# dougsouza/pytorch-sync-batchnorm-example

Hardware: AMD Instinct MI355X
Metric: images/sec (whole node) resnet50 SyncBN (higher is better)
Workload: dtype bf16; 1 GPU; model=resnet50, global_batch=512, per_gpu_batch=512, image=3x224x224, memory_format=channels_last, parallelism=dp1, impl=msbn, hip_graph=False, conv_autotune=False, fused_bn_act=True

## Files before the change

### msbn/models/resnet.py

```python

from typing import List, Type, Union

import torch
import torch.nn as nn

from msbn.nn import BatchNorm2d, SyncBatchNorm
from msbn.nn.fused import SyncBatchNormAct2d


def conv3x3(cin, cout, stride=1):
    return nn.Conv2d(cin, cout, 3, stride=stride, padding=1, bias=False)


def conv1x1(cin, cout, stride=1):
    return nn.Conv2d(cin, cout, 1, stride=stride, bias=False)


def _norm(planes, fused):
    return SyncBatchNorm(planes) if fused else BatchNorm2d(planes)


def _split(x):
    return x if isinstance(x, tuple) else (x, x)

# ... 77 lines not shown


class ResNet(nn.Module):
    def __init__(
        self,
        block: Type[Union[BasicBlock, Bottleneck]],
        layers: List[int],
        num_classes: int = 1000,
        in_chans: int = 3,
        fused: bool = False,
        fork_grads: bool = True,
    ):
        super().__init__()
        self.fused = fused
        self.fork_grads = fork_grads and fused
        self.inplanes = 64
        self.conv1 = nn.Conv2d(in_chans, 64, 7, stride=2, padding=3, bias=False)
        if fused:
            self.bn1 = SyncBatchNormAct2d(64, relu=True)
        else:
            self.bn1 = BatchNorm2d(64)
        self.relu = nn.ReLU(inplace=True)
        self.maxpool = nn.MaxPool2d(3, stride=2, padding=1)
        self.layer1 = self._make_layer(block, 64, layers[0])
        self.layer2 = self._make_layer(block, 128, layers[1], stride=2)
        self.layer3 = self._make_layer(block, 256, layers[2], stride=2)
        self.layer4 = self._make_layer(block, 512, layers[3], stride=2,
                                       fork_last=False)
        self.avgpool = nn.AdaptiveAvgPool2d(1)
        self.fc = nn.Linear(512 * block.expansion, num_classes)
# ... 10 lines not shown
            downsample = nn.Sequential(
                conv1x1(self.inplanes, planes * block.expansion, stride),
                _norm(planes * block.expansion, self.fused),
            )
        layers = [block(self.inplanes, planes, stride, downsample,
                        fused=self.fused, fork=fork[0])]
        self.inplanes = planes * block.expansion
        for i in range(1, blocks):
            layers.append(block(self.inplanes, planes, fused=self.fused,
                                fork=fork[i]))
        return nn.Sequential(*layers)

    def _stem(self, x):
        x = self.conv1(x)
        if self.fused:
            return self.maxpool(self.bn1(x))
        return self.maxpool(self.relu(self.bn1(x)))

    def forward_features(self, x):
        x = self._stem(x)
        c2 = self.layer1(x)
        c3 = self.layer2(c2)
        c4 = self.layer3(c3)
        c5 = self.layer4(c4)
        return _split(c2)[0], _split(c3)[0], _split(c4)[0], _split(c5)[0]

    def forward(self, x):
        _, _, _, c5 = self.forward_features(x)
        out = self.avgpool(c5).flatten(1)
        return self.fc(out)
# ... 13 lines not shown
```

### msbn/nn/fused.py

```python

from typing import Optional

import torch
import torch.distributed as dist

from msbn import ops
from msbn.nn.batchnorm import (SyncBatchNorm, _check_negative_slope,
                               _momentum_factor, _running_stats_forward)
from msbn.nn.functions import (_combined_view, _contig, _force_sync,
                               _match_layout, compute_sync_stats)


class SyncBatchNormActFunction(torch.autograd.Function):
    @staticmethod
    def forward(
        ctx,
        input: torch.Tensor,
        residual: Optional[torch.Tensor],
        weight: Optional[torch.Tensor],
        bias: Optional[torch.Tensor],
        running_mean: Optional[torch.Tensor],
        running_var: Optional[torch.Tensor],
        eps: float,
        momentum: float,
# ... 183 lines not shown
            else:
                grad_input, grad_res = ops.batch_norm_backward_elemt_act(
                    grad_output, input, residual, mean, invstd, weight, bias,
                    sum_dy, sum_dy_xmu, count_sum, relu, need_res_g, coefs,
                    slope,
                )
        return (
            grad_input if need_input_g else None,
            grad_res,
            grad_weight if need_weight_g else None,
            grad_bias if need_bias_g else None,
            None, None, None, None, None, None, None, None, None,
        )


class InPlaceSyncBatchNormActFunction(torch.autograd.Function):

    @staticmethod
    def forward(
        ctx,
        input: torch.Tensor,
        weight: torch.Tensor,
        bias: torch.Tensor,
        running_mean: Optional[torch.Tensor],
        running_var: Optional[torch.Tensor],
        eps: float,
        momentum: float,
        process_group,
        world_size: int,
        act: bool,
# ... 172 lines not shown
```

### msbn/ops/__init__.py

```python

from typing import Optional

import torch

from msbn.ops import _reference as _ref

_C = None
_C_IMPORT_ERROR: Optional[BaseException] = None
try:
    import os as _os

    if _os.environ.get("MSBN_AB_NONT", "0") == "1":
        from msbn import _C_nont as _C
    else:
        from msbn import _C as _C
except Exception as e:
    _C_IMPORT_ERROR = e


def hip_available() -> bool:
    return _C is not None


def _require_hip():
# ... 185 lines not shown
                                  relu_mask, want_res_grad, coefs=None,
                                  negative_slope: float = 0.0):
    if input.is_cuda:
        dx, dres = _require_hip().batch_norm_backward_elemt_act(
            grad_out, input, residual, mean, invstd, weight, bias, sum_dy,
            sum_dy_xmu, count, relu_mask, want_res_grad, coefs,
            negative_slope,
        )
        return dx, (dres if want_res_grad else None)
    return _ref.batch_norm_backward_elemt_act(
        grad_out, input, residual, mean, invstd, weight, bias, sum_dy,
        sum_dy_xmu, count, relu_mask, want_res_grad, negative_slope,
    )


def batch_norm_elemt_act_(input, weight, bias, mean, invstd, act: bool,
                          coefs=None, negative_slope: float = 0.0):
    if input.is_cuda:
        _require_hip().batch_norm_elemt_act_(
            input, weight, bias, mean, invstd, act, coefs, negative_slope
        )
        return input
    return _ref.batch_norm_elemt_act_(
        input, weight, bias, mean, invstd, act, negative_slope
    )


def batch_norm_backward_reduce_inplace(grad_out, output, invstd, weight, bias,
                                       act: bool, input_g, weight_g, bias_g,
                                       coefs=None,
# ... 51 lines not shown

def launch_plan(kind: str, input: torch.Tensor, others=(), coefs=None) -> dict:
    path, numbers = _require_hip().launch_plan(kind, input, list(others), coefs)
    plan = dict(numbers)
    plan["path"] = path
    if "multi_trip" in plan:
        plan["multi_trip"] = bool(plan["multi_trip"])
    return plan


__all__ = [
    "hip_available",
    "launch_plan",
    "bn_frozen_coefs",
    "batch_norm_frozen_backward_elemt",
    "batch_norm_elemt_act_",
    "batch_norm_backward_reduce_inplace",
    "batch_norm_backward_elemt_inplace",
    "batch_norm_elemt_act",
    "bn_make_coefs",
    "batch_norm_backward_reduce_act",
    "batch_norm_backward_elemt_act",
    "batch_norm_stats",
    "batch_norm_stats_packed",
    "batch_norm_gather_stats_with_counts",
    "batch_norm_gather_stats_packed",
    "batch_norm_elemt",
    "batch_norm_backward_reduce",
    "batch_norm_backward_elemt",
]
# ... 1 lines not shown
```

### msbn/ops/_reference.py

```python

from typing import Optional, Tuple

import torch


def _flatten_to_ncs(input: torch.Tensor) -> torch.Tensor:
    if input.dim() == 2:
        return input.unsqueeze(-1)
    return input.reshape(input.shape[0], input.shape[1], -1)


def batch_norm_stats(input: torch.Tensor, eps: float) -> Tuple[torch.Tensor, torch.Tensor]:
    x = _flatten_to_ncs(input)
    C = x.shape[1]
    n = x.shape[0] * x.shape[2]
    if n == 0:
        z = torch.zeros(C, dtype=torch.float32, device=input.device)
        return z, z.clone()
    xd = x.transpose(0, 1).reshape(C, -1).to(torch.float64)
    mean = xd.mean(dim=1)
    var = xd.var(dim=1, unbiased=False)
    invstd = torch.rsqrt(var + eps)
    return mean.to(torch.float32), invstd.to(torch.float32)

# ... 128 lines not shown

def batch_norm_backward_elemt_act(
    grad_out, input, residual, mean, invstd, weight, bias, sum_dy,
    sum_dy_xmu, count, relu_mask, want_res_grad, negative_slope: float = 0.0,
):
    g = _masked_grad(grad_out, input, residual, mean, invstd, weight, bias,
                     relu_mask, negative_slope)
    dx = batch_norm_backward_elemt(
        g, input, mean, invstd, weight, sum_dy, sum_dy_xmu, count
    )
    dres = g.to(grad_out.dtype) if want_res_grad else None
    return dx, dres



def _check_invertible(act: bool, negative_slope: float, name: str):
    if act and not negative_slope > 0.0:
        raise RuntimeError(
            f"{name}: the in-place path needs an invertible activation "
            "(identity, or LeakyReLU with negative_slope > 0); got "
            f"negative_slope={negative_slope}"
        )


def _slope32(negative_slope: float):
    s = torch.tensor(negative_slope, dtype=torch.float32)
    return s, 1.0 / s


def _invert_act(grad_out, output, act: bool, negative_slope: float):
# ... 144 lines not shown
```

### msbn/ops/csrc/bn_kernels.hip

```cpp
#include "bn_ops.hpp"
#include "common.hpp"

#include <ATen/ATen.h>
#include <c10/hip/HIPStream.h>

#include <algorithm>
#include <map>
#include <string>
#include <vector>

namespace msbn {

namespace {

template <typename T, int V>
__global__ void bn_stats_partial_nchw(const T* __restrict__ x,
                                      double* __restrict__ ws, int64_t N,
                                      int64_t C, int64_t S, int64_t chunkN,
                                      int64_t chunkS) {
  const int64_t c = blockIdx.x;
  const int64_t n0 = blockIdx.y * chunkN;
  const int64_t n1 = i64min(n0 + chunkN, N);
  const int64_t s0 = blockIdx.z * chunkS;
  const int64_t s1 = i64min(s0 + chunkS, S);
// ... 1375 lines not shown
      float g = to_f(nt_load1(&dy[e])), z;
      inv_act<ACT>(to_f(nt_load1(&y[e])), g, z, slope, inv_slope);
      nt_store1(&dx[e], from_f<T>(ca[c] * g + cb[c] * z + cd[c]));
    } else {
      Pack<T, V> pg = nt_load<T, V>(&dy[e]);
      Pack<T, V> py = nt_load<T, V>(&y[e]);
      Pack<float, V> pa = *reinterpret_cast<const Pack<float, V>*>(&ca[c]);
      Pack<float, V> pb = *reinterpret_cast<const Pack<float, V>*>(&cb[c]);
      Pack<float, V> pd = *reinterpret_cast<const Pack<float, V>*>(&cd[c]);
      Pack<T, V> po;
#pragma unroll
      for (int k = 0; k < V; ++k) {
        float g = to_f(pg.v[k]), z;
        inv_act<ACT>(to_f(py.v[k]), g, z, slope, inv_slope);
        po.v[k] = from_f<T>(pa.v[k] * g + pb.v[k] * z + pd.v[k]);
      }
      nt_store<T, V>(&dx[e], po);
    }
  }
}


struct Layout {
  bool nhwc;
  int64_t N, C, S;
  int64_t rows;
};

Layout get_layout(const at::Tensor& t) {
  Layout L{};
// ... 892 lines not shown
  });
  return {dx, dres};
}

at::Tensor batch_norm_backward_elemt(
    const at::Tensor& grad_out, const at::Tensor& input, const at::Tensor& mean,
    const at::Tensor& invstd, const c10::optional<at::Tensor>& weight,
    const at::Tensor& sum_dy, const at::Tensor& sum_dy_xmu,
    const at::Tensor& count) {
  return std::get<0>(batch_norm_backward_elemt_act(
      grad_out, input, c10::nullopt, mean, invstd, weight, c10::nullopt,
      sum_dy, sum_dy_xmu, count, false, false, c10::nullopt, 0.0));
}

namespace {
int inplace_act_mode(bool act, float slope, const char* name) {
  TORCH_CHECK(!act || slope > 0.f, name,
              ": the in-place path needs an invertible activation (identity, "
              "or LeakyReLU with negative_slope > 0); got negative_slope=",
              slope);
  return act ? kActLeaky : kActNone;
}

void check_same_dense(const at::Tensor& a, const at::Tensor& ref,
                      const char* what) {
  TORCH_CHECK(a.sizes() == ref.sizes() && a.strides() == ref.strides() &&
                  a.scalar_type() == ref.scalar_type() &&
                  a.device() == ref.device(),
              what, " must match the output's shape/strides/dtype/device");
}
// ... 580 lines not shown
  std::string path;

  if (kind == "fused_local") {
    if (!bn_fused_local_eligible(input, c10::nullopt, c10::nullopt,
                                 c10::nullopt, c10::nullopt))
      return {"ineligible", d};
    const int64_t C = input.size(1);
    const int64_t plane = input.numel() / C;
    const int64_t S = plane / input.size(0);
    d["V"] = pick_v(esize, ptrs, S);
    d["trips"] = cdiv(plane / d["V"], MSBN_BLOCK);
    d["blocks"] = C;
    return {"small_plane", d};
  }

  const Layout L = get_layout(input);
  if (kind == "stats" || kind == "bwd_reduce" ||
      kind == "bwd_reduce_inplace") {
    const ReducePlan p = plan_reduce(L, esize, ptrs);
    path = p.path == RedPath::Nhwc       ? "nhwc"
           : p.path == RedPath::NchwFlat ? "nchw_flat"
                                         : "nchw_vec";
    d["V"] = p.v;
    d["nchunks"] = p.nchunks;
    d["trips"] = p.trips;
    d["flush_every"] = p.flush_every;
    d["finalize_trips"] = cdiv(p.nchunks, MSBN_WAVE);
    if (p.path == RedPath::NchwVec) {
      d["chunkN"] = p.nchw.chunkN;
      d["chunkS"] = p.nchw.chunkS;
      d["nchunkS"] = p.nchw.grid.z;
    } else if (p.path == RedPath::NchwFlat) {
      d["chunk_len"] = p.flat.chunk_len;
    } else {
      d["chunk_rows"] = p.nhwc.chunk_rows;
      d["lpr"] = p.nhwc.lpr;
      d["ctiles"] = p.nhwc.grid.x;
    }
    return {path, d};
  }
  TORCH_CHECK(kind == "elemt" || kind == "bwd_elemt" ||
                  kind == "frozen_bwd_elemt" || kind == "elemt_inplace" ||
                  kind == "bwd_elemt_inplace",
              "launch_plan: unknown kind '", kind, "'");
  const ElemtPlan p = plan_elemt(L, input.numel(), esize, ptrs, coef);
  path = L.nhwc ? "nhwc" : (p.v == 1 ? "nchw_flat" : "nchw_vec");
  const int64_t threads = (int64_t)p.grid * MSBN_BLOCK;
  d["V"] = p.v;
  d["grid"] = p.grid;
  d["packs"] = p.packs;
  d["trips"] = cdiv(p.packs, threads);
  d["multi_trip"] = p.packs > threads ? 1 : 0;
  return {path, d};
}

}
```

### msbn/ops/csrc/bn_ops.hpp

```cpp
#pragma once

#include <ATen/ATen.h>

#include <map>
#include <string>
#include <tuple>
#include <vector>

namespace msbn {

std::tuple<at::Tensor, at::Tensor> batch_norm_stats(const at::Tensor& input,
                                                    double eps);

void batch_norm_stats_packed(const at::Tensor& input, double eps,
                             at::Tensor& out);

std::tuple<at::Tensor, at::Tensor> batch_norm_gather_stats_with_counts(
    const at::Tensor& mean_all, const at::Tensor& invstd_all,
    const c10::optional<at::Tensor>& running_mean,
    const c10::optional<at::Tensor>& running_var, double momentum, double eps,
    const at::Tensor& counts);

std::tuple<at::Tensor, at::Tensor, at::Tensor> batch_norm_gather_stats_packed(
    const at::Tensor& packed_all, const c10::optional<at::Tensor>& running_mean,
// ... 88 lines not shown
                           const at::Tensor& mean, const at::Tensor& invstd,
                           const c10::optional<at::Tensor>& weight,
                           const c10::optional<at::Tensor>& coefs,
                           bool relu_mask, bool want_res_grad, bool weight_g,
                           bool bias_g, double negative_slope);

std::tuple<at::Tensor, at::Tensor> batch_norm_backward_elemt_act(
    const at::Tensor& grad_out, const at::Tensor& input,
    const c10::optional<at::Tensor>& residual, const at::Tensor& mean,
    const at::Tensor& invstd, const c10::optional<at::Tensor>& weight,
    const c10::optional<at::Tensor>& bias, const at::Tensor& sum_dy,
    const at::Tensor& sum_dy_xmu, const at::Tensor& count, bool relu_mask,
    bool want_res_grad, const c10::optional<at::Tensor>& coefs_in,
    double negative_slope);

at::Tensor batch_norm_elemt_act_(at::Tensor& input,
                                 const c10::optional<at::Tensor>& weight,
                                 const c10::optional<at::Tensor>& bias,
                                 const at::Tensor& mean,
                                 const at::Tensor& invstd, bool act,
                                 const c10::optional<at::Tensor>& coefs_in,
                                 double negative_slope);

std::tuple<at::Tensor, at::Tensor, at::Tensor, at::Tensor>
batch_norm_backward_reduce_inplace(
    const at::Tensor& grad_out, const at::Tensor& output,
    const at::Tensor& invstd, const c10::optional<at::Tensor>& weight,
    const c10::optional<at::Tensor>& bias, bool act, bool input_g,
    bool weight_g, bool bias_g, const c10::optional<at::Tensor>& coefs_in,
    double negative_slope);
// ... 16 lines not shown
```

### msbn/ops/csrc/common.hpp

```cpp
#pragma once

#include <hip/hip_runtime.h>
#include <hip/hip_bf16.h>
#include <hip/hip_fp16.h>

#define MSBN_WAVE 64
#define MSBN_BLOCK 256

namespace msbn {

template <typename T, int V>
struct alignas(sizeof(T) * V) Pack {
  T v[V];
};

__device__ __forceinline__ float to_f(float x) { return x; }
__device__ __forceinline__ float to_f(__hip_bfloat16 x) {
  return __bfloat162float(x);
}
__device__ __forceinline__ float to_f(__half x) { return __half2float(x); }

template <typename T>
__device__ __forceinline__ T from_f(float x);
template <>
// ... 38 lines not shown
template <>
struct NTVec<16> {
  using type = int __attribute__((vector_size(16)));
};
template <>
struct NTVec<8> {
  using type = int __attribute__((vector_size(8)));
};
template <>
struct NTVec<4> {
  using type = int;
};
template <>
struct NTVec<2> {
  using type = short;
};

template <typename T, int V>
__device__ __forceinline__ Pack<T, V> nt_load(const T* p) {
#ifdef MSBN_DISABLE_NT
  return *reinterpret_cast<const Pack<T, V>*>(p);
#else
  using VT = typename NTVec<(int)sizeof(T) * V>::type;
  union {
    VT v;
    Pack<T, V> pk;
  } u;
  u.v = __builtin_nontemporal_load(reinterpret_cast<const VT*>(p));
  return u.pk;
#endif
// ... 97 lines not shown
```

### msbn/ops/csrc/module.cpp

```cpp
#include <torch/extension.h>

#include <torch/csrc/distributed/c10d/ProcessGroup.hpp>

#include "bn_ops.hpp"
#include "reducer.hpp"

PYBIND11_MODULE(TORCH_EXTENSION_NAME, m) {
  m.doc() = "msbn MI355X-native kernels + reducer";

  m.def("batch_norm_stats", &msbn::batch_norm_stats, py::arg("input"),
        py::arg("eps"));
  m.def("batch_norm_stats_packed", &msbn::batch_norm_stats_packed,
        py::arg("input"), py::arg("eps"), py::arg("out"));
  m.def("batch_norm_gather_stats_with_counts",
        &msbn::batch_norm_gather_stats_with_counts, py::arg("mean_all"),
        py::arg("invstd_all"), py::arg("running_mean"), py::arg("running_var"),
        py::arg("momentum"), py::arg("eps"), py::arg("counts"));
  m.def("batch_norm_gather_stats_packed",
        &msbn::batch_norm_gather_stats_packed, py::arg("packed_all"),
        py::arg("running_mean"), py::arg("running_var"), py::arg("momentum"),
        py::arg("eps"));
  m.def("batch_norm_gather_stats_packed_coefs",
        &msbn::batch_norm_gather_stats_packed_coefs, py::arg("packed_all"),
        py::arg("running_mean"), py::arg("running_var"), py::arg("momentum"),
// ... 22 lines not shown
        py::arg("coefs") = py::none(), py::arg("negative_slope") = 0.0);
  m.def("batch_norm_backward_reduce_act",
        &msbn::batch_norm_backward_reduce_act, py::arg("grad_out"),
        py::arg("input"), py::arg("residual"), py::arg("mean"),
        py::arg("invstd"), py::arg("weight"), py::arg("bias"),
        py::arg("relu_mask"), py::arg("input_g"), py::arg("weight_g"),
        py::arg("bias_g"), py::arg("coefs") = py::none(),
        py::arg("gm_out") = py::none(), py::arg("negative_slope") = 0.0,
        py::arg("grad_out2") = py::none());
  m.def("batch_norm_backward_elemt_act", &msbn::batch_norm_backward_elemt_act,
        py::arg("grad_out"), py::arg("input"), py::arg("residual"),
        py::arg("mean"), py::arg("invstd"), py::arg("weight"), py::arg("bias"),
        py::arg("sum_dy"), py::arg("sum_dy_xmu"), py::arg("count"),
        py::arg("relu_mask"), py::arg("want_res_grad"),
        py::arg("coefs") = py::none(), py::arg("negative_slope") = 0.0);

  m.def("batch_norm_elemt_act_", &msbn::batch_norm_elemt_act_,
        py::arg("input"), py::arg("weight"), py::arg("bias"), py::arg("mean"),
        py::arg("invstd"), py::arg("act"), py::arg("coefs") = py::none(),
        py::arg("negative_slope") = 0.0);
  m.def("batch_norm_backward_reduce_inplace",
        &msbn::batch_norm_backward_reduce_inplace, py::arg("grad_out"),
        py::arg("output"), py::arg("invstd"), py::arg("weight"),
        py::arg("bias"), py::arg("act"), py::arg("input_g"),
        py::arg("weight_g"), py::arg("bias_g"), py::arg("coefs") = py::none(),
        py::arg("negative_slope") = 0.0);
  m.def("batch_norm_backward_elemt_inplace",
        &msbn::batch_norm_backward_elemt_inplace, py::arg("grad_out"),
        py::arg("output"), py::arg("mean"), py::arg("invstd"),
        py::arg("weight"), py::arg("bias"), py::arg("sum_dy"),
// ... 71 lines not shown
```

Measured before the change: 9520 images/sec.

## Fuse stem BN+ReLU with 3x3 maxpool using argmax codes in forward and backward

```diff
diff --git a/msbn/models/resnet.py b/msbn/models/resnet.py
--- a/msbn/models/resnet.py
+++ b/msbn/models/resnet.py
@@ -5,7 +5,7 @@
 import torch.nn as nn
 
 from msbn.nn import BatchNorm2d, SyncBatchNorm
-from msbn.nn.fused import SyncBatchNormAct2d
+from msbn.nn.fused import SyncBatchNormAct2d, bn_act_maxpool
 
 
 def conv3x3(cin, cout, stride=1):
@@ -115,6 +115,7 @@
         super().__init__()
         self.fused = fused
         self.fork_grads = fork_grads and fused
+        self.stem_pool = fused
         self.inplanes = 64
         self.conv1 = nn.Conv2d(in_chans, 64, 7, stride=2, padding=3, bias=False)
         if fused:
@@ -155,6 +156,10 @@
     def _stem(self, x):
         x = self.conv1(x)
         if self.fused:
+            if (getattr(self, "stem_pool", True)
+                    and isinstance(self.bn1, SyncBatchNormAct2d)):
+                return bn_act_maxpool(self.bn1, self.maxpool, x,
+                                      fork=getattr(self, "fork_grads", False))
             return self.maxpool(self.bn1(x))
         return self.maxpool(self.relu(self.bn1(x)))
 
diff --git a/msbn/nn/fused.py b/msbn/nn/fused.py
--- a/msbn/nn/fused.py
+++ b/msbn/nn/fused.py
@@ -221,6 +221,155 @@
         )
 
 
+class SyncBatchNormActPoolFunction(torch.autograd.Function):
+
+    @staticmethod
+    def forward(
+        ctx,
+        input: torch.Tensor,
+        weight: Optional[torch.Tensor],
+        bias: Optional[torch.Tensor],
+        running_mean: Optional[torch.Tensor],
+        running_var: Optional[torch.Tensor],
+        eps: float,
+        momentum: float,
+        process_group,
+        world_size: int,
+        relu: bool,
+        negative_slope: float = 0.0,
+        fork: bool = False,
+    ):
+        if weight is not None:
+            weight = weight.contiguous()
+        if bias is not None:
+            bias = bias.contiguous()
+        use_sync = world_size > 1 or (
+            process_group is not None and _force_sync()
+        )
+        mean, invstd, count_sum, coefs = compute_sync_stats(
+            input, eps, momentum, running_mean, running_var,
+            process_group, world_size, weight, bias, want_coefs=True,
+        )
+        pooled, codes = ops.batch_norm_elemt_act_pool(
+            input, weight, bias, mean, invstd, relu, coefs, negative_slope
+        )
+        ctx.has_coefs = coefs is not None
+        saved = (input, codes, weight, bias, mean, invstd, count_sum)
+        ctx.save_for_backward(*(saved + ((coefs,) if ctx.has_coefs else ())))
+        ctx.relu = relu
+        ctx.negative_slope = negative_slope
+        ctx.process_group = process_group
+        ctx.use_sync = use_sync
+        if not fork:
+            return pooled
+        ctx.set_materialize_grads(False)
+        return pooled, pooled.detach()
+
+    @staticmethod
+    def backward(ctx, grad_output, grad_skip=None):
+        if grad_output is None:
+            grad_output, grad_skip = grad_skip, None
+        if grad_output is None:
+            return (None,) * 12
+        saved = ctx.saved_tensors
+        input, codes, weight, bias, mean, invstd, count_sum = saved[:7]
+        coefs = saved[7] if ctx.has_coefs else None
+        grad_output = _match_layout(grad_output, codes)
+        if grad_skip is not None:
+            grad_skip = _match_layout(grad_skip, codes)
+        relu, slope = ctx.relu, ctx.negative_slope
+        process_group = ctx.process_group
+        need_input_g = ctx.needs_input_grad[0]
+        need_weight_g = weight is not None and ctx.needs_input_grad[1]
+        need_bias_g = bias is not None and ctx.needs_input_grad[2]
+        C = int(input.shape[1])
+
+        sum_dy, sum_dy_xmu, grad_weight, grad_bias = (
+            ops.batch_norm_backward_reduce_act_pool(
+                grad_output, grad_skip, codes, input, mean, invstd, weight,
+                bias, relu, need_input_g, need_weight_g, need_bias_g, coefs,
+                slope,
+            )
+        )
+        grad_input = None
+        if need_input_g:
+            if ctx.use_sync:
+                combined, copied = _combined_view(sum_dy, sum_dy_xmu, C)
+                from msbn.utils import debug as _dbg
+                if _dbg.enabled():
+                    _dbg.verify_collective("syncbn.bwd.all_reduce",
+                                           combined, process_group)
+                dist.all_reduce(combined, dist.ReduceOp.SUM,
+                                group=process_group)
+                from msbn.utils.logging import comm_log
+                comm_log.record("all_reduce", combined.numel() * 4,
+                                f"syncbn bwd C={C}")
+                if copied:
+                    sum_dy, sum_dy_xmu = combined[:C], combined[C:]
+            grad_input = ops.batch_norm_backward_elemt_act_pool(
+                grad_output, grad_skip, codes, input, mean, invstd, weight,
+                bias, sum_dy, sum_dy_xmu, count_sum, relu, coefs, slope,
+            )
+        return (
+            grad_input,
+            grad_weight if need_weight_g else None,
+            grad_bias if need_bias_g else None,
+            None, None, None, None, None, None, None, None, None,
+        )
+
+
+def stem_pool_eligible(bn, pool, input: torch.Tensor) -> bool:
+    def _pair(v):
+        return tuple(v) if isinstance(v, (tuple, list)) else (v, v)
+
+    def _hooked(m):
+        return bool(m._forward_hooks or m._forward_pre_hooks
+                    or m._backward_hooks or m._backward_pre_hooks)
+
+    return (
+        type(bn) is SyncBatchNormAct2d
+        and not getattr(bn, "inplace", False)
+        and not _hooked(bn) and not _hooked(pool)
+        and (bn.training
+             or (bn.running_mean is None and bn.running_var is None))
+        and type(pool) is torch.nn.MaxPool2d
+        and _pair(pool.kernel_size) == (3, 3)
+        and _pair(pool.stride) == (2, 2)
+        and _pair(pool.padding) == (1, 1)
+        and _pair(pool.dilation) == (1, 1)
+        and not pool.ceil_mode and not pool.return_indices
+        and input.is_cuda and input.dim() == 4 and input.numel() > 0
+        and input.is_contiguous(memory_format=torch.channels_last)
+        and input.dtype in (torch.float32, torch.bfloat16, torch.float16)
+    )
+
+
+def bn_act_maxpool(bn, pool, input: torch.Tensor, fork: bool = False):
+    if not stem_pool_eligible(bn, pool, input):
+        y = pool(bn(input))
+        return (y, y) if fork else y
+    bn._check_input_dim(input)
+    bn._check_non_zero_input_channels(input)
+    if bn.training and bn.track_running_stats:
+        if bn.num_batches_tracked is not None:
+            bn.num_batches_tracked.add_(1)
+    factor = _momentum_factor(bn) if bn.training else (
+        bn.momentum if bn.momentum is not None else 0.0
+    )
+    process_group = None
+    world_size = 1
+    if dist.is_available() and dist.is_initialized():
+        process_group = bn.process_group or dist.group.WORLD
+        world_size = dist.get_world_size(process_group)
+    running_mean = bn.running_mean if bn.track_running_stats else None
+    running_var = bn.running_var if bn.track_running_stats else None
+    return SyncBatchNormActPoolFunction.apply(
+        input, bn.weight, bn.bias, running_mean, running_var, bn.eps, factor,
+        process_group, world_size, bn.relu,
+        getattr(bn, "negative_slope", 0.0), fork,
+    )
+
+
 class InPlaceSyncBatchNormActFunction(torch.autograd.Function):
 
     @staticmethod
diff --git a/msbn/ops/__init__.py b/msbn/ops/__init__.py
--- a/msbn/ops/__init__.py
+++ b/msbn/ops/__init__.py
@@ -223,6 +223,48 @@
     )
 
 
+def batch_norm_elemt_act_pool(input, weight, bias, mean, invstd, relu: bool,
+                              coefs=None, negative_slope: float = 0.0):
+    if input.is_cuda:
+        return _require_hip().batch_norm_elemt_act_pool(
+            input, weight, bias, mean, invstd, relu, coefs, negative_slope
+        )
+    return _ref.batch_norm_elemt_act_pool(
+        input, weight, bias, mean, invstd, relu, negative_slope
+    )
+
+
+def batch_norm_backward_reduce_act_pool(grad_out, grad_out2, codes, input,
+                                        mean, invstd, weight, bias, relu_mask,
+                                        input_g, weight_g, bias_g, coefs=None,
+                                        negative_slope: float = 0.0):
+    if input.is_cuda:
+        return _require_hip().batch_norm_backward_reduce_act_pool(
+            grad_out, grad_out2, codes, input, mean, invstd, weight, bias,
+            relu_mask, input_g, weight_g, bias_g, coefs, negative_slope,
+        )
+    return _ref.batch_norm_backward_reduce_act_pool(
+        grad_out, grad_out2, codes, input, mean, invstd, weight, bias,
+        relu_mask, input_g, weight_g, bias_g, negative_slope,
+    )
+
+
+def batch_norm_backward_elemt_act_pool(grad_out, grad_out2, codes, input,
+                                       mean, invstd, weight, bias, sum_dy,
+                                       sum_dy_xmu, count, relu_mask,
+                                       coefs=None,
+                                       negative_slope: float = 0.0):
+    if input.is_cuda:
+        return _require_hip().batch_norm_backward_elemt_act_pool(
+            grad_out, grad_out2, codes, input, mean, invstd, weight, bias,
+            sum_dy, sum_dy_xmu, count, relu_mask, coefs, negative_slope,
+        )
+    return _ref.batch_norm_backward_elemt_act_pool(
+        grad_out, grad_out2, codes, input, mean, invstd, weight, bias,
+        sum_dy, sum_dy_xmu, count, relu_mask, negative_slope,
+    )
+
+
 def batch_norm_elemt_act_(input, weight, bias, mean, invstd, act: bool,
                           coefs=None, negative_slope: float = 0.0):
     if input.is_cuda:
@@ -304,6 +346,9 @@
     "launch_plan",
     "bn_frozen_coefs",
     "batch_norm_frozen_backward_elemt",
+    "batch_norm_elemt_act_pool",
+    "batch_norm_backward_reduce_act_pool",
+    "batch_norm_backward_elemt_act_pool",
     "batch_norm_elemt_act_",
     "batch_norm_backward_reduce_inplace",
     "batch_norm_backward_elemt_inplace",
diff --git a/msbn/ops/_reference.py b/msbn/ops/_reference.py
--- a/msbn/ops/_reference.py
+++ b/msbn/ops/_reference.py
@@ -166,6 +166,106 @@
 
 
 
+def pool_out_size(size: int) -> int:
+    return (size - 1) // 2 + 1
+
+
+def _pooled_like(t: torch.Tensor, ref: torch.Tensor) -> torch.Tensor:
+    if ref.is_contiguous(memory_format=torch.channels_last):
+        return t.contiguous(memory_format=torch.channels_last)
+    return t.contiguous()
+
+
+def batch_norm_elemt_act_pool(input, weight, bias, mean, invstd, relu: bool,
+                              negative_slope: float = 0.0):
+    y = batch_norm_elemt_act(input, None, weight, bias, mean, invstd, relu,
+                             negative_slope)
+    N, C, H, W = y.shape
+    OH, OW = pool_out_size(H), pool_out_size(W)
+    yp = torch.nn.functional.pad(y.to(torch.float32), (1, 1, 1, 1),
+                                 value=float("-inf"))
+    best = torch.full((N, C, OH, OW), float("-inf"), dtype=torch.float32,
+                      device=y.device)
+    first_h = torch.zeros(OH, dtype=torch.uint8, device=y.device)
+    first_w = torch.zeros(OW, dtype=torch.uint8, device=y.device)
+    first_h[0] = 3
+    first_w[0] = 1
+    codes = (first_h.reshape(1, 1, OH, 1) + first_w.reshape(1, 1, 1, OW)
+             ).expand(N, C, OH, OW).clone()
+    for kh in range(3):
+        for kw in range(3):
+            val = yp[:, :, kh:kh + 2 * OH - 1:2, kw:kw + 2 * OW - 1:2]
+            upd = (val > best) | torch.isnan(val)
+            best = torch.where(upd, val, best)
+            codes = torch.where(upd, torch.full_like(codes, kh * 3 + kw),
+                                codes)
+    return (_pooled_like(best.to(input.dtype), input),
+            _pooled_like(codes, input))
+
+
+def pool_codes_to_indices(codes: torch.Tensor, H: int, W: int) -> torch.Tensor:
+    OH, OW = codes.shape[2], codes.shape[3]
+    c = codes.to(torch.int64)
+    oh = torch.arange(OH, device=codes.device).reshape(1, 1, OH, 1)
+    ow = torch.arange(OW, device=codes.device).reshape(1, 1, 1, OW)
+    return (2 * oh - 1 + c // 3) * W + (2 * ow - 1 + c % 3)
+
+
+def pool_gather_grad(grad_out, grad_out2, codes, input):
+    g = grad_out
+    if grad_out2 is not None:
+        g = grad_out + grad_out2
+    g = g.to(torch.float32)
+    N, C, H, W = input.shape
+    OH, OW = codes.shape[2], codes.shape[3]
+    full = torch.zeros((N, C, H, W), dtype=torch.float32,
+                       device=input.device)
+    for kh in (2, 1, 0):
+        lo_h = 1 if kh == 0 else 0
+        hi_h = min(OH - 1, (H - kh) // 2)
+        for kw in (2, 1, 0):
+            lo_w = 1 if kw == 0 else 0
+            hi_w = min(OW - 1, (W - kw) // 2)
+            if hi_h < lo_h or hi_w < lo_w:
+                continue
+            sel = (slice(None), slice(None), slice(lo_h, hi_h + 1),
+                   slice(lo_w, hi_w + 1))
+            part = torch.where(codes[sel] == kh * 3 + kw, g[sel],
+                               torch.zeros_like(g[sel]))
+            h0, w0 = 2 * lo_h - 1 + kh, 2 * lo_w - 1 + kw
+            dst = (slice(None), slice(None),
+                   slice(h0, h0 + 2 * (hi_h - lo_h) + 1, 2),
+                   slice(w0, w0 + 2 * (hi_w - lo_w) + 1, 2))
+            full[dst] = full[dst] + part
+    full = full.to(input.dtype)
+    if input.is_contiguous(memory_format=torch.channels_last):
+        full = full.contiguous(memory_format=torch.channels_last)
+    return full
+
+
+def batch_norm_backward_reduce_act_pool(
+    grad_out, grad_out2, codes, input, mean, invstd, weight, bias, relu_mask,
+    input_g, weight_g, bias_g, negative_slope: float = 0.0,
+):
+    g = pool_gather_grad(grad_out, grad_out2, codes, input)
+    return batch_norm_backward_reduce_act(
+        g, input, None, mean, invstd, weight, bias, relu_mask, input_g,
+        weight_g, bias_g, None, negative_slope,
+    )
+
+
+def batch_norm_backward_elemt_act_pool(
+    grad_out, grad_out2, codes, input, mean, invstd, weight, bias, sum_dy,
+    sum_dy_xmu, count, relu_mask, negative_slope: float = 0.0,
+):
+    g = pool_gather_grad(grad_out, grad_out2, codes, input)
+    return batch_norm_backward_elemt_act(
+        g, input, None, mean, invstd, weight, bias, sum_dy, sum_dy_xmu,
+        count, relu_mask, False, negative_slope,
+    )[0]
+
+
+
 def _check_invertible(act: bool, negative_slope: float, name: str):
     if act and not negative_slope > 0.0:
         raise RuntimeError(
diff --git a/msbn/ops/csrc/bn_kernels.hip b/msbn/ops/csrc/bn_kernels.hip
--- a/msbn/ops/csrc/bn_kernels.hip
+++ b/msbn/ops/csrc/bn_kernels.hip
@@ -1413,6 +1413,300 @@
         float g = to_f(pg.v[k]), z;
         inv_act<ACT>(to_f(py.v[k]), g, z, slope, inv_slope);
         po.v[k] = from_f<T>(pa.v[k] * g + pb.v[k] * z + pd.v[k]);
+      }
+      nt_store<T, V>(&dx[e], po);
+    }
+  }
+}
+
+#ifndef MSBN_POOL_FWD_NT
+#define MSBN_POOL_FWD_NT 0
+#endif
+#ifndef MSBN_POOL_GATHER_NT
+#define MSBN_POOL_GATHER_NT 0
+#endif
+
+template <typename T, int V, bool NT>
+__device__ __forceinline__ Pack<T, V> pool_load(const T* p) {
+  if (NT) return nt_load<T, V>(p);
+  return *reinterpret_cast<const Pack<T, V>*>(p);
+}
+
+template <typename T, int V, int ACT>
+__global__ void bn_elemt_pool_nhwc(const T* __restrict__ x,
+                                   T* __restrict__ y,
+                                   uint8_t* __restrict__ codes,
+                                   const float* __restrict__ scale,
+                                   const float* __restrict__ shift,
+                                   int64_t total, int64_t C, int H, int W,
+                                   int OH, int OW, float slope) {
+  const int64_t stride = (int64_t)gridDim.x * blockDim.x;
+  for (int64_t i = (int64_t)blockIdx.x * blockDim.x + threadIdx.x;
+       i * V < total; i += stride) {
+    const int64_t e = i * V;
+    const uint32_t pix = (uint32_t)(e / C);
+    const int64_t c = e - (int64_t)pix * C;
+    const uint32_t t = pix / (uint32_t)OW;
+    const int ow = (int)(pix - t * (uint32_t)OW);
+    const int n = (int)(t / (uint32_t)OH);
+    const int oh = (int)(t - (uint32_t)n * (uint32_t)OH);
+    const int h0 = 2 * oh - 1, w0 = 2 * ow - 1;
+    Pack<float, V> ps, pb;
+    if (V == 1) {
+      ps.v[0] = scale[c];
+      pb.v[0] = shift[c];
+    } else {
+      ps = *reinterpret_cast<const Pack<float, V>*>(&scale[c]);
+      pb = *reinterpret_cast<const Pack<float, V>*>(&shift[c]);
+    }
+    float best[V];
+    uint8_t code[V];
+    const uint8_t first = (uint8_t)((h0 < 0 ? 3 : 0) + (w0 < 0 ? 1 : 0));
+#pragma unroll
+    for (int k = 0; k < V; ++k) {
+      best[k] = -INFINITY;
+      code[k] = first;
+    }
+#pragma unroll
+    for (int kh = 0; kh < 3; ++kh) {
+      const int h = h0 + kh;
+      if (h < 0 || h >= H) continue;
+#pragma unroll
+      for (int kw = 0; kw < 3; ++kw) {
+        const int w = w0 + kw;
+        if (w < 0 || w >= W) continue;
+        const int64_t off = (((int64_t)n * H + h) * W + w) * C + c;
+        const Pack<T, V> px = pool_load<T, V, MSBN_POOL_FWD_NT>(&x[off]);
+#pragma unroll
+        for (int k = 0; k < V; ++k) {
+          float z = to_f(px.v[k]) * ps.v[k] + pb.v[k];
+          z = act_fwd<ACT>(z, slope);
+          const float val = to_f(from_f<T>(z));
+          if (val > best[k] || val != val) {
+            best[k] = val;
+            code[k] = (uint8_t)(kh * 3 + kw);
+          }
+        }
+      }
+    }
+    Pack<T, V> py;
+    Pack<uint8_t, V> pc;
+#pragma unroll
+    for (int k = 0; k < V; ++k) {
+      py.v[k] = from_f<T>(best[k]);
+      pc.v[k] = code[k];
+    }
+    nt_store<T, V>(&y[e], py);
+    nt_store<uint8_t, V>(&codes[e], pc);
+  }
+}
+
+template <typename T, int V, bool DY2>
+__device__ __forceinline__ void pool_gather(const T* __restrict__ dy,
+                                            const T* __restrict__ dy2,
+                                            const uint8_t* __restrict__ codes,
+                                            int n, int h, int w, int64_t c,
+                                            int64_t C, int OH, int OW,
+                                            float (&g)[V]) {
+#pragma unroll
+  for (int k = 0; k < V; ++k) g[k] = 0.f;
+  const int oh0 = h >> 1, ow0 = w >> 1;
+  const int noh = ((h & 1) && oh0 + 1 < OH) ? 2 : 1;
+  const bool two_w = (w & 1) && ow0 + 1 < OW;
+  const int ow1 = two_w ? ow0 + 1 : ow0;
+  const int kw0 = w - (2 * ow0 - 1);
+  for (int a = 0; a < noh; ++a) {
+    const int oh = oh0 + a;
+    const int kh3 = (h - (2 * oh - 1)) * 3;
+    const uint8_t want0 = (uint8_t)(kh3 + kw0);
+    const uint8_t want1 = two_w ? (uint8_t)kh3 : (uint8_t)0xff;
+    const int64_t row = ((int64_t)n * OH + oh) * OW;
+    const int64_t off0 = (row + ow0) * C + c;
+    const int64_t off1 = (row + ow1) * C + c;
+    constexpr bool GNT = MSBN_POOL_GATHER_NT;
+    const Pack<uint8_t, V> pc0 = pool_load<uint8_t, V, GNT>(&codes[off0]);
+    const Pack<T, V> pg0 = pool_load<T, V, GNT>(&dy[off0]);
+    Pack<T, V> ph0, ph1;
+    if (DY2) ph0 = pool_load<T, V, GNT>(&dy2[off0]);
+    Pack<uint8_t, V> pc1;
+    Pack<T, V> pg1;
+#pragma unroll
+    for (int k = 0; k < V; ++k) {
+      pc1.v[k] = 0xff;
+      pg1.v[k] = from_f<T>(0.f);
+      if (DY2) ph1.v[k] = from_f<T>(0.f);
+    }
+    if (two_w) {
+      pc1 = pool_load<uint8_t, V, GNT>(&codes[off1]);
+      pg1 = pool_load<T, V, GNT>(&dy[off1]);
+      if (DY2) ph1 = pool_load<T, V, GNT>(&dy2[off1]);
+    }
+#pragma unroll
+    for (int k = 0; k < V; ++k) {
+      const float g0 = DY2 ? fork_grad(pg0.v[k], ph0.v[k]) : to_f(pg0.v[k]);
+      const float g1 = DY2 ? fork_grad(pg1.v[k], ph1.v[k]) : to_f(pg1.v[k]);
+      if (pc0.v[k] == want0) g[k] += g0;
+      if (pc1.v[k] == want1) g[k] += g1;
+    }
+  }
+#pragma unroll
+  for (int k = 0; k < V; ++k) g[k] = to_f(from_f<T>(g[k]));
+}
+
+template <typename T, int V, int ACT, bool DY2>
+__global__ void bn_bwd_reduce_pool_partial_nhwc(
+    const T* __restrict__ dy, const T* __restrict__ dy2,
+    const uint8_t* __restrict__ codes, const T* __restrict__ x,
+    const float* __restrict__ mean, const float* __restrict__ scale,
+    const float* __restrict__ shift, double* __restrict__ ws, int64_t rows,
+    int64_t C, int64_t chunk_rows, int lpr, int H, int W, int OH, int OW,
+    float slope) {
+  const int rpi = blockDim.x / lpr;
+  const int lane = threadIdx.x % lpr;
+  const int rowoff = threadIdx.x / lpr;
+  const bool active = rowoff < rpi;
+  const int64_t c = (int64_t)blockIdx.x * lpr * V + (int64_t)lane * V;
+  const bool inb = active && (c + V <= C);
+
+  AccPair acc[V];
+  float m[V], scv[V], shv[V];
+#pragma unroll
+  for (int k = 0; k < V; ++k) m[k] = scv[k] = shv[k] = 0.f;
+  if (inb) {
+#pragma unroll
+    for (int k = 0; k < V; ++k) {
+      m[k] = mean[c + k];
+      if (ACT) {
+        scv[k] = scale[c + k];
+        shv[k] = shift[c + k];
+      }
+    }
+    const int64_t r0 = (int64_t)blockIdx.y * chunk_rows;
+    const int64_t r1 = i64min(r0 + chunk_rows, rows);
+    int n = 0, h = 0, w = 0;
+    if (r0 + rowoff < r1) {
+      const uint32_t r = (uint32_t)(r0 + rowoff);
+      const uint32_t t = r / (uint32_t)W;
+      w = (int)(r - t * (uint32_t)W);
+      n = (int)(t / (uint32_t)H);
+      h = (int)(t - (uint32_t)n * (uint32_t)H);
+    }
+    int since_flush = 0;
+    for (int64_t r = r0 + rowoff; r < r1; r += rpi) {
+      float g[V];
+      pool_gather<T, V, DY2>(dy, dy2, codes, n, h, w, c, C, OH, OW, g);
+      Pack<T, V> px = nt_load<T, V>(&x[r * C + c]);
+#pragma unroll
+      for (int k = 0; k < V; ++k) {
+        const float xv = to_f(px.v[k]);
+        if (ACT) {
+          float z = scv[k] * xv + shv[k];
+          g[k] = act_gate<ACT>(z, g[k], slope);
+        }
+        acc[k].add2(g[k], g[k] * (xv - m[k]));
+      }
+      if (++since_flush == MSBN_ACC_FLUSH) {
+#pragma unroll
+        for (int k = 0; k < V; ++k) acc[k].flush();
+        since_flush = 0;
+      }
+      w += rpi;
+      while (w >= W) {
+        w -= W;
+        if (++h == H) {
+          h = 0;
+          ++n;
+        }
+      }
+    }
+  }
+  double a[V], b[V];
+#pragma unroll
+  for (int k = 0; k < V; ++k) {
+    acc[k].flush();
+    a[k] = acc[k].a;
+    b[k] = acc[k].b;
+  }
+  __shared__ double sdata[MSBN_BLOCK * V * 2];
+#pragma unroll
+  for (int k = 0; k < V; ++k) {
+    sdata[k * MSBN_BLOCK + threadIdx.x] = a[k];
+    sdata[(V + k) * MSBN_BLOCK + threadIdx.x] = b[k];
+  }
+  for (int st = 1; st < rpi; st <<= 1) {
+    __syncthreads();
+    if (active && (rowoff & ((st << 1) - 1)) == 0 && rowoff + st < rpi) {
+      const int other = threadIdx.x + st * lpr;
+#pragma unroll
+      for (int k = 0; k < V; ++k) {
+        sdata[k * MSBN_BLOCK + threadIdx.x] += sdata[k * MSBN_BLOCK + other];
+        sdata[(V + k) * MSBN_BLOCK + threadIdx.x] +=
+            sdata[(V + k) * MSBN_BLOCK + other];
+      }
+    }
+  }
+  __syncthreads();
+  if (rowoff == 0 && c < C) {
+    const int64_t chunk = blockIdx.y;
+#pragma unroll
+    for (int k = 0; k < V; ++k) {
+      if (c + k < C) {
+        double* out = ws + ((c + k) * gridDim.y + chunk) * 2;
+        out[0] = sdata[k * MSBN_BLOCK + threadIdx.x];
+        out[1] = sdata[(V + k) * MSBN_BLOCK + threadIdx.x];
+      }
+    }
+  }
+}
+
+template <typename T, int V, int ACT, bool DY2>
+__global__ void bn_bwd_elemt_pool_nhwc(
+    const T* __restrict__ dy, const T* __restrict__ dy2,
+    const uint8_t* __restrict__ codes, const T* __restrict__ x,
+    T* __restrict__ dx, const float* __restrict__ ca,
+    const float* __restrict__ cb, const float* __restrict__ cd,
+    const float* __restrict__ scale, const float* __restrict__ shift,
+    int64_t total, int64_t C, int H, int W, int OH, int OW, float slope) {
+  const int64_t stride = (int64_t)gridDim.x * blockDim.x;
+  for (int64_t i = (int64_t)blockIdx.x * blockDim.x + threadIdx.x;
+       i * V < total; i += stride) {
+    const int64_t e = i * V;
+    const uint32_t pix = (uint32_t)(e / C);
+    const int64_t c = e - (int64_t)pix * C;
+    const uint32_t t = pix / (uint32_t)W;
+    const int w = (int)(pix - t * (uint32_t)W);
+    const int n = (int)(t / (uint32_t)H);
+    const int h = (int)(t - (uint32_t)n * (uint32_t)H);
+    float g[V];
+    pool_gather<T, V, DY2>(dy, dy2, codes, n, h, w, c, C, OH, OW, g);
+    if (V == 1) {
+      const float xv = to_f(nt_load1(&x[e]));
+      float gv = g[0];
+      if (ACT) {
+        float z = scale[c] * xv + shift[c];
+        gv = act_gate<ACT>(z, gv, slope);
+      }
+      nt_store1(&dx[e], from_f<T>(ca[c] * gv + cb[c] * xv + cd[c]));
+    } else {
+      Pack<T, V> px = nt_load<T, V>(&x[e]);
+      Pack<float, V> pa = *reinterpret_cast<const Pack<float, V>*>(&ca[c]);
+      Pack<float, V> pb = *reinterpret_cast<const Pack<float, V>*>(&cb[c]);
+      Pack<float, V> pd = *reinterpret_cast<const Pack<float, V>*>(&cd[c]);
+      Pack<float, V> psc, psh;
+      if (ACT) {
+        psc = *reinterpret_cast<const Pack<float, V>*>(&scale[c]);
+        psh = *reinterpret_cast<const Pack<float, V>*>(&shift[c]);
+      }
+      Pack<T, V> po;
+#pragma unroll
+      for (int k = 0; k < V; ++k) {
+        float gv = g[k];
+        const float xv = to_f(px.v[k]);
+        if (ACT) {
+          float z = psc.v[k] * xv + psh.v[k];
+          gv = act_gate<ACT>(z, gv, slope);
+        }
+        po.v[k] = from_f<T>(pa.v[k] * gv + pb.v[k] * xv + pd.v[k]);
       }
       nt_store<T, V>(&dx[e], po);
     }
@@ -2335,6 +2629,263 @@
 }
 
 namespace {
+struct PoolGeom {
+  int H, W, OH, OW;
+};
+
+Layout pool_layout(const at::Tensor& x, const char* op) {
+  TORCH_CHECK(x.dim() == 4 &&
+                  x.is_contiguous(at::MemoryFormat::ChannelsLast),
+              op, ": input must be a dense 4-D channels-last tensor");
+  Layout L{};
+  L.nhwc = true;
+  L.N = x.size(0);
+  L.C = x.size(1);
+  L.S = x.size(2) * x.size(3);
+  L.rows = L.N * L.S;
+  return L;
+}
+
+PoolGeom pool_geom(const at::Tensor& x, const Layout& L, const char* op) {
+  TORCH_CHECK(L.rows < (int64_t)INT32_MAX, op, ": N*H*W must be below 2^31");
+  PoolGeom g{};
+  g.H = (int)x.size(2);
+  g.W = (int)x.size(3);
+  g.OH = (g.H - 1) / 2 + 1;
+  g.OW = (g.W - 1) / 2 + 1;
+  return g;
+}
+
+void check_pooled(const at::Tensor& t, const at::Tensor& x, const PoolGeom& g,
+                  at::ScalarType dtype, const char* op, const char* what) {
+  TORCH_CHECK(t.dim() == 4 && t.size(0) == x.size(0) &&
+                  t.size(1) == x.size(1) && t.size(2) == g.OH &&
+                  t.size(3) == g.OW && t.scalar_type() == dtype &&
+                  t.device() == x.device() &&
+                  t.is_contiguous(at::MemoryFormat::ChannelsLast),
+              op, ": ", what, " must be a channels-last [N, C, OH, OW] ",
+              dtype, " tensor on the input's device");
+}
+}
+
+std::tuple<at::Tensor, at::Tensor> batch_norm_elemt_act_pool(
+    const at::Tensor& input, const c10::optional<at::Tensor>& weight,
+    const c10::optional<at::Tensor>& bias, const at::Tensor& mean,
+    const at::Tensor& invstd, bool relu,
+    const c10::optional<at::Tensor>& coefs_in, double negative_slope) {
+  const Layout L = pool_layout(input, "bn_elemt_pool");
+  TORCH_CHECK(input.numel() > 0, "bn_elemt_pool: empty input");
+  const PoolGeom g = pool_geom(input, L, "bn_elemt_pool");
+  const float slope = (float)negative_slope;
+  const int act = act_mode(relu, slope);
+  auto out = at::empty({input.size(0), L.C, g.OH, g.OW},
+                       input.options().memory_format(
+                           at::MemoryFormat::ChannelsLast));
+  auto codes = at::empty_like(out, out.options().dtype(at::kByte));
+  auto stream = cur_stream();
+  auto coefs = coefs_in.has_value()
+                   ? *coefs_in
+                   : make_fwd_coefs(mean, invstd, weight, bias, L.C);
+  float* scale = coefs.data_ptr<float>();
+  float* shift = scale + L.C;
+  const int64_t total = out.numel();
+  MSBN_DISPATCH_FLOAT_TYPES(input.scalar_type(), "bn_elemt_pool", [&] {
+    const native_t* x =
+        reinterpret_cast<const native_t*>(input.data_ptr<scalar_t>());
+    native_t* y = reinterpret_cast<native_t*>(out.data_ptr<scalar_t>());
+    uint8_t* cp = codes.data_ptr<uint8_t>();
+    constexpr int VMAX = 16 / (int)sizeof(native_t);
+    const ElemtPlan plan =
+        plan_elemt(L, total, (int)sizeof(native_t), {x, y, cp}, scale);
+    MSBN_DISPATCH_V(plan.v, VMAX, [&] {
+      constexpr int VK = VV * (int)sizeof(native_t) <= 16 ? VV : 1;
+      MSBN_DISPATCH_ACT(act, ACT_, [&] {
+        hipLaunchKernelGGL((bn_elemt_pool_nhwc<native_t, VK, ACT_>),
+                           dim3(plan.grid), dim3(MSBN_BLOCK), 0, stream, x, y,
+                           cp, scale, shift, total, L.C, g.H, g.W, g.OH, g.OW,
+                           slope);
+      });
+    });
+  });
+  return {out, codes};
+}
+
+std::tuple<at::Tensor, at::Tensor, at::Tensor, at::Tensor>
+batch_norm_backward_reduce_act_pool(
+    const at::Tensor& grad_out, const c10::optional<at::Tensor>& grad_out2,
+    const at::Tensor& codes, const at::Tensor& input, const at::Tensor& mean,
+    const at::Tensor& invstd, const c10::optional<at::Tensor>& weight,
+    const c10::optional<at::Tensor>& bias, bool relu_mask, bool input_g,
+    bool weight_g, bool bias_g, const c10::optional<at::Tensor>& coefs_in,
+    double negative_slope) {
+  const Layout L = pool_layout(input, "bn_bwd_reduce_pool");
+  TORCH_CHECK(input.numel() > 0, "bn_bwd_reduce_pool: empty input");
+  const PoolGeom g = pool_geom(input, L, "bn_bwd_reduce_pool");
+  const float slope = (float)negative_slope;
+  const int act = act_mode(relu_mask, slope);
+  check_pooled(grad_out, input, g, input.scalar_type(), "bn_bwd_reduce_pool",
+               "grad_out");
+  const bool has_dy2 = grad_out2.has_value();
+  if (has_dy2)
+    check_pooled(*grad_out2, input, g, input.scalar_type(),
+                 "bn_bwd_reduce_pool", "grad_out2");
+  check_pooled(codes, input, g, at::kByte, "bn_bwd_reduce_pool", "codes");
+  auto f32 = input.options().dtype(at::kFloat);
+  auto combined = at::empty({2 * L.C}, f32);
+  auto sum_dy = combined.narrow(0, 0, L.C);
+  auto sum_dy_xmu = combined.narrow(0, L.C, L.C);
+  const auto wtype =
+      weight.has_value() ? weight->scalar_type() : input.scalar_type();
+  auto wopts = input.options().dtype(wtype);
+  at::Tensor grad_weight, grad_bias;
+  if (weight_g) grad_weight = at::empty({L.C}, wopts);
+  if (bias_g) grad_bias = at::empty({L.C}, wopts);
+
+  float* scale = nullptr;
+  float* shift = nullptr;
+  at::Tensor coefs;
+  if (relu_mask) {
+    coefs = coefs_in.has_value()
+                ? *coefs_in
+                : make_fwd_coefs(mean, invstd, weight, bias, L.C);
+    scale = coefs.data_ptr<float>();
+    shift = scale + L.C;
+  }
+
+  auto stream = cur_stream();
+  MSBN_DISPATCH_FLOAT_TYPES(input.scalar_type(), "bn_bwd_reduce_pool", [&] {
+    const native_t* x =
+        reinterpret_cast<const native_t*>(input.data_ptr<scalar_t>());
+    const native_t* dy =
+        reinterpret_cast<const native_t*>(grad_out.data_ptr<scalar_t>());
+    const native_t* dy2 =
+        has_dy2 ? reinterpret_cast<const native_t*>(grad_out2->data_ptr())
+                : nullptr;
+    const uint8_t* cp = codes.data_ptr<uint8_t>();
+    constexpr int VMAX = 16 / (int)sizeof(native_t);
+    const ReducePlan plan =
+        plan_reduce(L, (int)sizeof(native_t), {x, dy, dy2, cp});
+    const int nchunks = plan.nchunks;
+    const auto& ng = plan.nhwc;
+    at::Tensor ws = at::empty({(int64_t)nchunks * L.C * 2},
+                              input.options().dtype(at::kDouble));
+    MSBN_DISPATCH_V(plan.v, VMAX, [&] {
+      constexpr int VK = VV * (int)sizeof(native_t) <= 16 ? VV : 1;
+      MSBN_DISPATCH_ACT(act, ACT_, [&] {
+        MSBN_DISPATCH_BOOL(has_dy2, DY2_, [&] {
+          hipLaunchKernelGGL(
+              (bn_bwd_reduce_pool_partial_nhwc<native_t, VK, ACT_, DY2_>),
+              ng.grid, dim3(MSBN_BLOCK), 0, stream, dy, dy2, cp, x,
+              mean.data_ptr<float>(), scale, shift, ws.data_ptr<double>(),
+              L.rows, L.C, ng.chunk_rows, ng.lpr, g.H, g.W, g.OH, g.OW,
+              slope);
+        });
+      });
+    });
+    const int fgrid = (int)cdiv(L.C, kFinalizeWavesPerBlock);
+    MSBN_DISPATCH_RSTAT(wtype, "bn_bwd_reduce_pool", [&] {
+      rstat_t* gw = weight_g ? reinterpret_cast<rstat_t*>(grad_weight.data_ptr())
+                             : nullptr;
+      rstat_t* gb =
+          bias_g ? reinterpret_cast<rstat_t*>(grad_bias.data_ptr()) : nullptr;
+      hipLaunchKernelGGL((bn_bwd_reduce_finalize<rstat_t>), dim3(fgrid),
+                         dim3(MSBN_BLOCK), 0, stream, ws.data_ptr<double>(),
+                         nchunks, L.C, invstd.data_ptr<float>(),
+                         sum_dy.data_ptr<float>(),
+                         sum_dy_xmu.data_ptr<float>(), gw, gb);
+    });
+  });
+  (void)input_g;
+  return {sum_dy, sum_dy_xmu, grad_weight, grad_bias};
+}
+
+at::Tensor batch_norm_backward_elemt_act_pool(
+    const at::Tensor& grad_out, const c10::optional<at::Tensor>& grad_out2,
+    const at::Tensor& codes, const at::Tensor& input, const at::Tensor& mean,
+    const at::Tensor& invstd, const c10::optional<at::Tensor>& weight,
+    const c10::optional<at::Tensor>& bias, const at::Tensor& sum_dy,
+    const at::Tensor& sum_dy_xmu, const at::Tensor& count, bool relu_mask,
+    const c10::optional<at::Tensor>& coefs_in, double negative_slope) {
+  const Layout L = pool_layout(input, "bn_bwd_elemt_pool");
+  TORCH_CHECK(input.numel() > 0, "bn_bwd_elemt_pool: empty input");
+  const PoolGeom g = pool_geom(input, L, "bn_bwd_elemt_pool");
+  const float slope = (float)negative_slope;
+  const int act = act_mode(relu_mask, slope);
+  check_pooled(grad_out, input, g, input.scalar_type(), "bn_bwd_elemt_pool",
+               "grad_out");
+  const bool has_dy2 = grad_out2.has_value();
+  if (has_dy2)
+    check_pooled(*grad_out2, input, g, input.scalar_type(),
+                 "bn_bwd_elemt_pool", "grad_out2");
+  check_pooled(codes, input, g, at::kByte, "bn_bwd_elemt_pool", "codes");
+  auto dx = at::empty_like(input);
+  at::Tensor count_sum;
+  if (count.numel() == 1 && count.scalar_type() == at::kFloat) {
+    count_sum = count;
+  } else {
+    count_sum = count.to(at::kFloat).sum().reshape({1});
+  }
+  auto stream = cur_stream();
+  auto f32 = input.options().dtype(at::kFloat);
+  auto coefs = at::empty({3 * L.C}, f32);
+  float* ca = coefs.data_ptr<float>();
+  float* cb = ca + L.C;
+  float* cd = cb + L.C;
+  const int cgrid = (int)cdiv(L.C, MSBN_BLOCK);
+  const auto wtype =
+      weight.has_value() ? weight->scalar_type() : at::kFloat;
+  MSBN_DISPATCH_RSTAT(wtype, "bn_bwd_elemt_pool", [&] {
+    const rstat_t* w =
+        weight.has_value()
+            ? reinterpret_cast<const rstat_t*>(weight->data_ptr())
+            : nullptr;
+    hipLaunchKernelGGL((bn_affine_bwd<rstat_t>), dim3(cgrid), dim3(MSBN_BLOCK),
+                       0, stream, mean.data_ptr<float>(),
+                       invstd.data_ptr<float>(), w, sum_dy.data_ptr<float>(),
+                       sum_dy_xmu.data_ptr<float>(),
+                       count_sum.data_ptr<float>(), L.C, ca, cb, cd);
+  });
+  float* scale = nullptr;
+  float* shift = nullptr;
+  at::Tensor fcoefs;
+  if (relu_mask) {
+    fcoefs = coefs_in.has_value()
+                 ? *coefs_in
+                 : make_fwd_coefs(mean, invstd, weight, bias, L.C);
+    scale = fcoefs.data_ptr<float>();
+    shift = scale + L.C;
+  }
+  const int64_t total = input.numel();
+  MSBN_DISPATCH_FLOAT_TYPES(input.scalar_type(), "bn_bwd_elemt_pool", [&] {
+    const native_t* x =
+        reinterpret_cast<const native_t*>(input.data_ptr<scalar_t>());
+    const native_t* dy =
+        reinterpret_cast<const native_t*>(grad_out.data_ptr<scalar_t>());
+    const native_t* dy2 =
+        has_dy2 ? reinterpret_cast<const native_t*>(grad_out2->data_ptr())
+                : nullptr;
+    const uint8_t* cp = codes.data_ptr<uint8_t>();
+    native_t* o = reinterpret_cast<native_t*>(dx.data_ptr<scalar_t>());
+    constexpr int VMAX = 16 / (int)sizeof(native_t);
+    const ElemtPlan plan = plan_elemt(L, total, (int)sizeof(native_t),
+                                      {x, dy, dy2, cp, o}, scale);
+    MSBN_DISPATCH_V(plan.v, VMAX, [&] {
+      constexpr int VK = VV * (int)sizeof(native_t) <= 16 ? VV : 1;
+      MSBN_DISPATCH_ACT(act, ACT_, [&] {
+        MSBN_DISPATCH_BOOL(has_dy2, DY2_, [&] {
+          hipLaunchKernelGGL(
+              (bn_bwd_elemt_pool_nhwc<native_t, VK, ACT_, DY2_>),
+              dim3(plan.grid), dim3(MSBN_BLOCK), 0, stream, dy, dy2, cp, x, o,
+              ca, cb, cd, scale, shift, total, L.C, g.H, g.W, g.OH, g.OW,
+              slope);
+        });
+      });
+    });
+  });
+  return dx;
+}
+
+namespace {
 int inplace_act_mode(bool act, float slope, const char* name) {
   TORCH_CHECK(!act || slope > 0.f, name,
               ": the in-place path needs an invertible activation (identity, "
@@ -2945,9 +3496,12 @@
     return {"small_plane", d};
   }
 
-  const Layout L = get_layout(input);
+  const bool pool_kind = kind == "elemt_pool" || kind == "bwd_reduce_pool" ||
+                         kind == "bwd_elemt_pool";
+  const Layout L =
+      pool_kind ? pool_layout(input, "launch_plan") : get_layout(input);
   if (kind == "stats" || kind == "bwd_reduce" ||
-      kind == "bwd_reduce_inplace") {
+      kind == "bwd_reduce_inplace" || kind == "bwd_reduce_pool") {
     const ReducePlan p = plan_reduce(L, esize, ptrs);
     path = p.path == RedPath::Nhwc       ? "nhwc"
            : p.path == RedPath::NchwFlat ? "nchw_flat"
@@ -2972,9 +3526,15 @@
   }
   TORCH_CHECK(kind == "elemt" || kind == "bwd_elemt" ||
                   kind == "frozen_bwd_elemt" || kind == "elemt_inplace" ||
-                  kind == "bwd_elemt_inplace",
+                  kind == "bwd_elemt_inplace" || kind == "elemt_pool" ||
+                  kind == "bwd_elemt_pool",
               "launch_plan: unknown kind '", kind, "'");
-  const ElemtPlan p = plan_elemt(L, input.numel(), esize, ptrs, coef);
+  int64_t total = input.numel();
+  if (kind == "elemt_pool") {
+    const PoolGeom g = pool_geom(input, L, "launch_plan");
+    total = input.size(0) * L.C * g.OH * g.OW;
+  }
+  const ElemtPlan p = plan_elemt(L, total, esize, ptrs, coef);
   path = L.nhwc ? "nhwc" : (p.v == 1 ? "nchw_flat" : "nchw_vec");
   const int64_t threads = (int64_t)p.grid * MSBN_BLOCK;
   d["V"] = p.v;
diff --git a/msbn/ops/csrc/bn_ops.hpp b/msbn/ops/csrc/bn_ops.hpp
--- a/msbn/ops/csrc/bn_ops.hpp
+++ b/msbn/ops/csrc/bn_ops.hpp
@@ -126,6 +126,29 @@
     bool want_res_grad, const c10::optional<at::Tensor>& coefs_in,
     double negative_slope);
 
+std::tuple<at::Tensor, at::Tensor> batch_norm_elemt_act_pool(
+    const at::Tensor& input, const c10::optional<at::Tensor>& weight,
+    const c10::optional<at::Tensor>& bias, const at::Tensor& mean,
+    const at::Tensor& invstd, bool relu,
+    const c10::optional<at::Tensor>& coefs_in, double negative_slope);
+
+std::tuple<at::Tensor, at::Tensor, at::Tensor, at::Tensor>
+batch_norm_backward_reduce_act_pool(
+    const at::Tensor& grad_out, const c10::optional<at::Tensor>& grad_out2,
+    const at::Tensor& codes, const at::Tensor& input, const at::Tensor& mean,
+    const at::Tensor& invstd, const c10::optional<at::Tensor>& weight,
+    const c10::optional<at::Tensor>& bias, bool relu_mask, bool input_g,
+    bool weight_g, bool bias_g, const c10::optional<at::Tensor>& coefs_in,
+    double negative_slope);
+
+at::Tensor batch_norm_backward_elemt_act_pool(
+    const at::Tensor& grad_out, const c10::optional<at::Tensor>& grad_out2,
+    const at::Tensor& codes, const at::Tensor& input, const at::Tensor& mean,
+    const at::Tensor& invstd, const c10::optional<at::Tensor>& weight,
+    const c10::optional<at::Tensor>& bias, const at::Tensor& sum_dy,
+    const at::Tensor& sum_dy_xmu, const at::Tensor& count, bool relu_mask,
+    const c10::optional<at::Tensor>& coefs_in, double negative_slope);
+
 at::Tensor batch_norm_elemt_act_(at::Tensor& input,
                                  const c10::optional<at::Tensor>& weight,
                                  const c10::optional<at::Tensor>& bias,
diff --git a/msbn/ops/csrc/common.hpp b/msbn/ops/csrc/common.hpp
--- a/msbn/ops/csrc/common.hpp
+++ b/msbn/ops/csrc/common.hpp
@@ -76,6 +76,10 @@
 template <>
 struct NTVec<2> {
   using type = short;
+};
+template <>
+struct NTVec<1> {
+  using type = char;
 };
 
 template <typename T, int V>
diff --git a/msbn/ops/csrc/module.cpp b/msbn/ops/csrc/module.cpp
--- a/msbn/ops/csrc/module.cpp
+++ b/msbn/ops/csrc/module.cpp
@@ -60,6 +60,25 @@
         py::arg("sum_dy"), py::arg("sum_dy_xmu"), py::arg("count"),
         py::arg("relu_mask"), py::arg("want_res_grad"),
         py::arg("coefs") = py::none(), py::arg("negative_slope") = 0.0);
+
+  m.def("batch_norm_elemt_act_pool", &msbn::batch_norm_elemt_act_pool,
+        py::arg("input"), py::arg("weight"), py::arg("bias"), py::arg("mean"),
+        py::arg("invstd"), py::arg("relu"), py::arg("coefs") = py::none(),
+        py::arg("negative_slope") = 0.0);
+  m.def("batch_norm_backward_reduce_act_pool",
+        &msbn::batch_norm_backward_reduce_act_pool, py::arg("grad_out"),
+        py::arg("grad_out2"), py::arg("codes"), py::arg("input"),
+        py::arg("mean"), py::arg("invstd"), py::arg("weight"), py::arg("bias"),
+        py::arg("relu_mask"), py::arg("input_g"), py::arg("weight_g"),
+        py::arg("bias_g"), py::arg("coefs") = py::none(),
+        py::arg("negative_slope") = 0.0);
+  m.def("batch_norm_backward_elemt_act_pool",
+        &msbn::batch_norm_backward_elemt_act_pool, py::arg("grad_out"),
+        py::arg("grad_out2"), py::arg("codes"), py::arg("input"),
+        py::arg("mean"), py::arg("invstd"), py::arg("weight"), py::arg("bias"),
+        py::arg("sum_dy"), py::arg("sum_dy_xmu"), py::arg("count"),
+        py::arg("relu_mask"), py::arg("coefs") = py::none(),
+        py::arg("negative_slope") = 0.0);
 
   m.def("batch_norm_elemt_act_", &msbn::batch_norm_elemt_act_,
         py::arg("input"), py::arg("weight"), py::arg("bias"), py::arg("mean"),
```

After: 9737 images/sec, median of 6. +2.3%, better.
